# debbiemarkslab/EVcouplings

Hardware: NVIDIA H100
Metric: PLM gradient evals/s as N*L^2*q cell-ops/s (higher is better)
Workload: dtype f32 parameters/accumulation; tensor-core products as bf16 hi+lo pairs (16 mantissa bits)

## Files before the change

evcouplings_b200/csrc/api.cu:

```cuda
#include "../../include/evcplm.h"

#include <stdlib.h>

#include <new>
#include <string>
#include <vector>

#include "common.cuh"
#include "internal.h"

namespace evc {
static thread_local std::string g_err;
void set_error(const std::string &msg) { g_err = msg; }
}

using namespace evc;

static cudaStream_t as_stream(void *s) { return reinterpret_cast<cudaStream_t>(s); }

extern "C" {

int evc_abi_version(void) { return EVCPLM_ABI_VERSION; }

const char *evc_last_error(void) { return g_err.c_str(); }
// ... 241 lines not shown
    float *gJ = d_g + (int64_t)g.L * g.q;
    if ((!tc || (!tcf && !tcff)) && ensure_gather(h)) return 1;
    if (prof) EVC_CUDA(cudaEventRecord(h->ev[0], st));
    if (tcff) {
        if (plm_tcff_expand(g, h->tcff, d_x, h->d_wp_hi, h->d_wp_lo, single, st)) return 1;
        if (prof) EVC_CUDA(cudaEventRecord(h->ev[1], st));
        if (plm_tcff_forward(g, h->tcff, h->tcff_maps, d_x, h->d_msa4, h->d_wts, h->d_rt_hi, h->d_rt_lo, h->tc.Kp,
                             h->d_gh_part3, h->d_fx_part3, single, st))
            return 1;
        if (prof) {
            EVC_CUDA(cudaEventRecord(h->ev[2], st));
            EVC_CUDA(cudaEventRecord(h->ev[3], st));
        }
        if (plm_tc_backward(g, h->tc, h->tc_maps, h->d_Gd, single, st)) return 1;
        if (prof) EVC_CUDA(cudaEventRecord(h->ev[4], st));
        if (plm_tc_finalize_pairs(g, h->tc, h->d_Gd, gJ, 1.0f, st)) return 1;
        if (plm_finalize_fields_n(g, h->d_gh_part3, h->d_fx_part3, d_g, d_fx, h->tcff.ntile_part, st)) return 1;
    } else if (tcf) {
        if (plm_tcf_expand(g, h->tcf, d_x, h->d_wt_hi, h->d_wt_lo, single, st)) return 1;
        if (prof) EVC_CUDA(cudaEventRecord(h->ev[1], st));
        if (plm_tcf_logits(g, h->tcf, h->tcf_maps, h->d_zt, single, st)) return 1;
        if (prof) EVC_CUDA(cudaEventRecord(h->ev[2], st));
        if (plm_tcf_softmax(g, h->tcf, h->d_zt, d_x, h->d_msa4, h->d_wts, h->d_rt_hi, rt_lo, h->tc.Kp,
                            h->d_gh_part2, h->d_fx_part2, st))
            return 1;
        if (prof) EVC_CUDA(cudaEventRecord(h->ev[3], st));
        if (plm_tc_backward(g, h->tc, h->tc_maps, h->d_Gd, single, st)) return 1;
        if (prof) EVC_CUDA(cudaEventRecord(h->ev[4], st));
        if (plm_tc_finalize_pairs(g, h->tc, h->d_Gd, gJ, 1.0f, st)) return 1;
        if (plm_finalize_fields_n(g, h->d_gh_part2, h->d_fx_part2, d_g, d_fx, h->tcf.ntiles_s, st)) return 1;
    } else {
        if (plm_expand(g, d_x, h->d_W, st)) return 1;
        if (!tc) EVC_CUDA(cudaMemsetAsync(h->d_G, 0, (size_t)g.w_floats() * sizeof(float), st));
        if (prof) EVC_CUDA(cudaEventRecord(h->ev[1], st));
        if (plm_forward(g, h->d_W, d_x, h->d_msa4, h->d_wts, h->d_R, tc ? h->d_rt_hi : nullptr,
                        tc ? h->d_rt_lo : nullptr, h->tc.Kp, h->d_gh_part, h->d_fx_part, st))
            return 1;
        if (prof) {
            EVC_CUDA(cudaEventRecord(h->ev[2], st));
            EVC_CUDA(cudaEventRecord(h->ev[3], st));
        }
        if (tc) {
            if (plm_tc_backward(g, h->tc, h->tc_maps, h->d_Gd, single, st)) return 1;
            if (prof) EVC_CUDA(cudaEventRecord(h->ev[4], st));
            if (plm_tc_finalize_pairs(g, h->tc, h->d_Gd, gJ, 1.0f, st)) return 1;
            if (plm_finalize_fields(g, h->d_gh_part, h->d_fx_part, d_g, d_fx, st)) return 1;
        } else {
            if (plm_backward(g, h->d_R, h->d_perm, h->d_bstart, h->d_G, st)) return 1;
            if (prof) EVC_CUDA(cudaEventRecord(h->ev[4], st));
            if (plm_finalize(g, h->d_G, h->d_gh_part, h->d_fx_part, d_g, gJ, d_fx, 1.0f, st)) return 1;
        }
    }
    if (prof) {
        EVC_CUDA(cudaEventRecord(h->ev[5], st));
        h->ev_valid = true;
    }
    return 0;
}

int evc_plm_set_backward(evc_plm_t *h, int32_t mode)
{
    if (!h) { set_error("evc_plm_set_backward: null handle"); return 1; }
    if (mode != 0 && mode != 1) { set_error("evc_plm_set_backward: mode must be 0 (gather) or 1 (tensor core)"); return 1; }
    EVC_CUDA(cudaSetDevice(h->device));
    if (mode == 1 && !h->d_xt) {
        plm_tc_geometry(h->g, h->tc);
        const PlmTcGeom &t = h->tc;
        const size_t xb = (size_t)t.Mp * t.Kp * 2, rb = (size_t)t.Np * t.Kp * 2;
        if (cudaMalloc(&h->d_xt, xb) != cudaSuccess || cudaMalloc(&h->d_rt_hi, rb) != cudaSuccess ||
            cudaMalloc(&h->d_rt_lo, rb) != cudaSuccess ||
            cudaMalloc(&h->d_Gd, (size_t)t.Mp * t.Np * sizeof(float)) != cudaSuccess) {
            set_error(std::string("evc_plm_set_backward: device allocation failed: ") +
                      cudaGetErrorString(cudaGetLastError()));
            return 1;
        }
        EVC_CUDA(cudaMemset(h->d_rt_hi, 0, rb));
        EVC_CUDA(cudaMemset(h->d_rt_lo, 0, rb));
        EVC_CUDA(cudaMemset(h->d_Gd, 0, (size_t)t.Mp * t.Np * sizeof(float)));
        if (plm_tc_build_xt(h->g, t, h->d_msa4, h->d_xt, 0)) return 1;
        EVC_CUDA(cudaDeviceSynchronize());
        h->tc_maps = aligned_alloc(64, round_up((int64_t)plm_tc_map_bytes(), 64));
        if (!h->tc_maps) { set_error("evc_plm_set_backward: out of host memory"); return 1; }
        if (plm_tc_make_maps(t, h->d_xt, h->d_rt_hi, h->d_rt_lo, h->tc_maps)) return 1;
    }
    h->bwd_mode = mode;
    return 0;
}

int evc_plm_set_forward(evc_plm_t *h, int32_t mode)
{
    if (!h) { set_error("evc_plm_set_forward: null handle"); return 1; }
    if (mode < 0 || mode > 2) {
        set_error("evc_plm_set_forward: mode must be 0 (gather), 1 (tensor core) or 2 (tensor core, fused softmax)");
// ... 100 lines not shown
    EVC_CUDA(cudaStreamSynchronize(0));
    return 0;
}

int evc_plm_weighted_counts(evc_plm_t *h, float *d_fi_counts, float *d_fij_counts, void *stream)
{
    if (!h || !d_fi_counts || !d_fij_counts) { set_error("evc_plm_weighted_counts: null pointer"); return 1; }
    cudaStream_t st = as_stream(stream);
    const PlmGeom &g = h->g;
    if (h->bwd_mode == 1 && h->d_gh_part2) {
        const int ntiles = h->tcf.ntiles_s;
        if (plm_tc_onehot_residual(g, ntiles, h->d_msa4, h->d_wts, h->d_rt_hi, h->d_rt_lo, h->tc.Kp, h->d_gh_part2,
                                   h->d_fx_part2, st))
            return 1;
        if (plm_tc_backward(g, h->tc, h->tc_maps, h->d_Gd, 0, st)) return 1;
        if (plm_tc_finalize_pairs(g, h->tc, h->d_Gd, d_fij_counts, 0.5f, st)) return 1;
        return plm_finalize_fields_n(g, h->d_gh_part2, nullptr, d_fi_counts, nullptr, ntiles, st);
    }
    if (ensure_gather(h)) return 1;
    EVC_CUDA(cudaMemsetAsync(h->d_G, 0, (size_t)g.w_floats() * sizeof(float), st));
    if (plm_onehot_residual(g, h->d_msa4, h->d_wts, h->d_R, h->d_gh_part, st)) return 1;
    if (plm_backward(g, h->d_R, h->d_perm, h->d_bstart, h->d_G, st)) return 1;
    return plm_finalize(g, h->d_G, h->d_gh_part, nullptr, d_fi_counts, d_fij_counts, nullptr, 0.5f, st);
}

int evc_ec_scores(const float *d_J_tri, const float *d_fij_tri, const float *d_fi, int32_t L, int32_t q,
                  float *d_fn_raw, float *d_fn_zero_sum, float *d_mi, void *stream)
{
    if (!d_J_tri) { set_error("evc_ec_scores: null pointer"); return 1; }
    return ec_scores(d_J_tri, d_fij_tri, d_fi, L, q, d_fn_raw, d_fn_zero_sum, d_mi, as_stream(stream));
}
// ... 47 lines not shown
```

evcouplings_b200/csrc/internal.h:

```cpp
#pragma once
#include <cuda_runtime.h>
#include <stdint.h>

namespace evc {

int64_t hamming_plane_words(int64_t N, int L);
int64_t hamming_num_tiles(int64_t N);
int hamming_pack(const uint8_t *d_codes, int64_t N, int L, uint32_t *d_planes, cudaStream_t st);
int hamming_count_tiles(const uint32_t *d_planes, int64_t N, int L, int min_identical,
                        int64_t tile_begin, int64_t tile_end, int *d_counts, cudaStream_t st);

int identities_to_seq(const uint8_t *d_codes, const uint8_t *d_seq, int64_t N, int L, int *d_out, cudaStream_t st);

struct PlmGeom {
    int64_t N;
    int L;
    int Lp;
    int q;
    int QB;
    int S;
    int gap_code;
    int64_t Nr;
    int64_t Nld;
    int L4;
// ... 19 lines not shown
                const float *d_wts, float *d_R, void *d_rt_hi, void *d_rt_lo, int64_t Kp, float *d_gh_part,
                double *d_fx_part, cudaStream_t st);
int plm_onehot_residual(const PlmGeom &g, const uint32_t *d_msa4, const float *d_wts, float *d_R,
                        float *d_gh_part, cudaStream_t st);
int plm_backward(const PlmGeom &g, const float *d_R, const uint32_t *d_perm, const uint16_t *d_bstart,
                 float *d_G, cudaStream_t st);
int plm_finalize(const PlmGeom &g, const float *d_G, const float *d_gh_part, const double *d_fx_part,
                 float *d_gh, float *d_gJ, double *d_fx, float scale_pair, cudaStream_t st);
int plm_add_reg(const PlmGeom &g, const float *d_x, float *d_g, double *d_fx, float lambda_h,
                float lambda_J, cudaStream_t st);

struct PlmTcGeom {
    int64_t Mp;
    int64_t Np;
    int64_t Kp;
};
void plm_tc_geometry(const PlmGeom &g, PlmTcGeom &t);
size_t plm_tc_map_bytes();
int plm_tc_build_xt(const PlmGeom &g, const PlmTcGeom &t, const uint32_t *d_msa4, void *d_xt, cudaStream_t st);
int plm_tc_make_maps(const PlmTcGeom &t, void *d_xt, void *d_rt_hi, void *d_rt_lo, void *maps_out_host);
int plm_tc_backward(const PlmGeom &g, const PlmTcGeom &t, const void *maps_host, float *d_Gd, int single,
                    cudaStream_t st);
int plm_tc_onehot_residual(const PlmGeom &g, int ntiles, const uint32_t *d_msa4, const float *d_wts, void *d_rt_hi,
                           void *d_rt_lo, int64_t Kp, float *d_gh_part, double *d_fx_part, cudaStream_t st);
int plm_tc_finalize_pairs(const PlmGeom &g, const PlmTcGeom &t, const float *d_Gd, float *d_gJ, float scale,
                          cudaStream_t st);
struct PlmTcfGeom {
    int64_t Mp;
    int64_t Kw;
    int64_t Ns;
    int64_t Xrows;
    int ntiles_s;
};
void plm_tcf_geometry(const PlmGeom &g, PlmTcfGeom &t);
int plm_tcf_build_x(const PlmGeom &g, const PlmTcfGeom &t, const uint32_t *d_msa4, void *d_x1h, cudaStream_t st);
int plm_tcf_make_maps(const PlmTcfGeom &t, void *d_wt_hi, void *d_wt_lo, void *d_x1h, void *maps_out_host);
int plm_tcf_expand(const PlmGeom &g, const PlmTcfGeom &t, const float *d_x, void *d_wt_hi, void *d_wt_lo,
                   int single, cudaStream_t st);
int plm_tcf_logits(const PlmGeom &g, const PlmTcfGeom &t, const void *maps_host, float *d_zt, int single,
                   cudaStream_t st);
int plm_tcf_softmax(const PlmGeom &g, const PlmTcfGeom &t, const float *d_zt, const float *d_x,
// ... 88 lines not shown
```

evcouplings_b200/csrc/plm_tc.cu:

```cuda
#include <cuda.h>
#include <cuda_bf16.h>

#include <stdlib.h>

#include <algorithm>

#include "common.cuh"
#include "internal.h"

namespace evc {

constexpr int TC_BM = 128;
constexpr int TC_BN = 192;
constexpr int TC_BK = 64;
constexpr int TC_MAX_STAGES = 8;
constexpr int TC_A_BYTES = TC_BM * TC_BK * 2;
constexpr int TC_B_BYTES = TC_BN * TC_BK * 2;
constexpr int TC_SMEM_LIMIT = 232448;
constexpr int TC_SMEM_HEAD = 2048;
constexpr int TC_THREADS = 384;
constexpr int TC_CONSUMERS = 256;
constexpr int TC_K_CHUNK = 32;
constexpr int TC_REG_PRODUCER = 40;
constexpr int TC_REG_CONSUMER = 232;

__device__ __forceinline__ void mbar_wait_bounded(uint64_t *bar, uint32_t parity)
{
    uint32_t done = 0;
    for (uint64_t it = 0; it < (1ull << 31); it++) {
        asm volatile(
            "{\n.reg .pred p;\n"
            "mbarrier.try_wait.parity.shared::cta.b64 p, [%1], %2;\n"
            "selp.u32 %0, 1, 0, p;\n}\n"
            : "=r"(done)
            : "r"(smem_u32(bar)), "r"(parity)
            : "memory");
        if (done) return;
// ... 188 lines not shown
{
    if (threadIdx.x == 0) {
        for (int s = 0; s < n_stages; s++) {
            mbar_init(&l.full[s], 1);
            mbar_init(&l.empty[s], TC_CONSUMERS);
        }
        mbar_fence_init();
    }
    __syncthreads();
}

template <int SPLIT_A, int SINGLE>
__global__ void __launch_bounds__(TC_THREADS, 1)
tc_gemm_kernel(const __grid_constant__ CUtensorMap tm0, const __grid_constant__ CUtensorMap tm1,
               const __grid_constant__ CUtensorMap tm2, float *__restrict__ D, int64_t ldd, int m_tiles, int n_tiles,
               int num_kb, int k_chunk, int mgroup, int n_stages)
{
    constexpr int BYTES0 = TC_A_BYTES;
    constexpr int BYTES1 = TC_B_BYTES;
    constexpr int BYTES2 = SPLIT_A ? TC_A_BYTES : TC_B_BYTES;
    constexpr int stage_bytes = BYTES0 + BYTES1 + (SINGLE ? 0 : BYTES2);
    extern __shared__ unsigned char smem_dyn[];
    const TcSmem l = tc_smem_layout(smem_dyn);
    int m_tile, n_tile;
    decode_tile(blockIdx.x, m_tiles, n_tiles, mgroup, m_tile, n_tile);
    tc_init_barriers(l, n_stages);

    if (threadIdx.x < 128) {
        setmaxnreg_dec<TC_REG_PRODUCER>();
        if (threadIdx.x == 0) {
            const uint64_t keep = l2_policy_evict_last();
            int s = 0;
            uint32_t ph = 0;
            for (int kb = 0; kb < num_kb; kb++) {
                mbar_wait_bounded(&l.empty[s], ph ^ 1u);
                unsigned char *st = l.ring + s * stage_bytes;
                mbar_expect_tx(&l.full[s], (uint32_t)stage_bytes);
                if (SPLIT_A) {
                    tma_load_2d_hint(st, &tm0, kb * TC_BK, m_tile * TC_BM, &l.full[s], keep);
                    tma_load_2d(st + BYTES0, &tm2, kb * TC_BK, n_tile * TC_BN, &l.full[s]);
                    if (!SINGLE) tma_load_2d_hint(st + BYTES0 + BYTES1, &tm1, kb * TC_BK, m_tile * TC_BM, &l.full[s], keep);
                } else {
                    tma_load_2d(st, &tm0, kb * TC_BK, m_tile * TC_BM, &l.full[s]);
                    tma_load_2d(st + BYTES0, &tm1, kb * TC_BK, n_tile * TC_BN, &l.full[s]);
                    if (!SINGLE) tma_load_2d(st + BYTES0 + BYTES1, &tm2, kb * TC_BK, n_tile * TC_BN, &l.full[s]);
                }
                if (++s == n_stages) { s = 0; ph ^= 1u; }
            }
        }
    } else {
        setmaxnreg_inc<TC_REG_CONSUMER>();
        const int cw = (threadIdx.x >> 7) - 1;
        constexpr uint64_t OFF1 = (uint64_t)(BYTES0 >> 4), OFF2 = (uint64_t)((BYTES0 + BYTES1) >> 4);
        const uint64_t arow = (uint64_t)((cw * 64 * TC_BK * 2) >> 4);
        const uint64_t desc0 = make_desc_sw128(l.ring);
        float acc[TC_BN / 2], sum[TC_BN / 2];
#pragma unroll
        for (int u = 0; u < TC_BN / 2; u++) acc[u] = 0.f;
        const int n_chunks = (num_kb + k_chunk - 1) / k_chunk;
        int s = 0;
        uint32_t ph = 0;
        for (int c = 0; c < n_chunks; c++) {
            const int kb0 = c * k_chunk, kb1 = min(num_kb, kb0 + k_chunk);
            if (SPLIT_A) tc_mainloop<TC_BN>(acc, l.full, l.empty, s, ph, n_stages, stage_bytes, kb0, kb1, desc0,
                                            arow, OFF1, OFF2 + arow, OFF1, !SINGLE);
            else tc_mainloop<TC_BN>(acc, l.full, l.empty, s, ph, n_stages, stage_bytes, kb0, kb1, desc0,
                                    arow, OFF1, arow, OFF2, !SINGLE);
#pragma unroll
            for (int u = 0; u < TC_BN / 2; u++) sum[u] = (c == 0) ? acc[u] : sum[u] + acc[u];
        }
        const int t = threadIdx.x & 127;
        const int64_t row = (int64_t)m_tile * TC_BM + cw * 64 + (t >> 5) * 16 + ((t & 31) >> 2);
        float *out = D + row * ldd + (int64_t)n_tile * TC_BN + 2 * (t & 3);
#pragma unroll
        for (int c8 = 0; c8 < TC_BN / 8; c8++) {
            __stcs(reinterpret_cast<float2 *>(out + 8 * c8), make_float2(sum[4 * c8], sum[4 * c8 + 1]));
            __stcs(reinterpret_cast<float2 *>(out + 8 * ldd + 8 * c8), make_float2(sum[4 * c8 + 2], sum[4 * c8 + 3]));
        }
    }
}

constexpr int TF_BN = 176;
constexpr int TF_SITES = 8;
constexpr int TF_B_BYTES = TF_BN * TC_BK * 2;
constexpr int TF_PITCH = TF_BN + 1;

template <int SINGLE>
__global__ void __launch_bounds__(TC_THREADS, 1)
// ... 97 lines not shown
                if (n < g.N) {
                    const int64_t off = ((int64_t)i * q + a) * Kp + n;
                    const __nv_bfloat16 hi = __float2bfloat16_rn(rr);
                    Rt_hi[off] = hi;
                    if (!SINGLE) Rt_lo[off] = __float2bfloat16_rn(rr - __bfloat162float(hi));
                }
            }
            const float tot = warp_sum(rr);
            if (lane == 0) ghp[a] = (a < q) ? tot : 0.f;
        }
        const double fw = warp_sum(fx_local);
        if (lane == 0) fx_part[(int64_t)i * ntile_part + m_tile * 4 + quad] = fw;
    }
}

__global__ void expand_tcf_kernel(const float *__restrict__ x, __nv_bfloat16 *__restrict__ Wp_hi,
                                  __nv_bfloat16 *__restrict__ Wp_lo, int L, int q, int64_t ldw, int single)
{
    const int i = blockIdx.y, j = blockIdx.x;
    if (j <= i) return;
    const float *J = x + (int64_t)L * q + ((int64_t)i * (2 * L - i - 1) / 2 + (j - i - 1)) * q * q;
    const int64_t ri = (int64_t)(i / TF_SITES) * TF_BN + ((i % TF_SITES) / 4) * 88 + (i % 4) * 21;
    const int64_t rj = (int64_t)(j / TF_SITES) * TF_BN + ((j % TF_SITES) / 4) * 88 + (j % 4) * 21;
    for (int e = threadIdx.x; e < q * q; e += blockDim.x) {
        const int a = e / q, b = e - a * q;
        const float v = J[e];
        const __nv_bfloat16 hi = __float2bfloat16_rn(v);
        const __nv_bfloat16 lo = __float2bfloat16_rn(v - __bfloat162float(hi));
        const int64_t p1 = (ri + a) * ldw + (j * q + b);
        const int64_t p2 = (rj + b) * ldw + (i * q + a);
        Wp_hi[p1] = hi;
        Wp_hi[p2] = hi;
        if (!single) { Wp_lo[p1] = lo; Wp_lo[p2] = lo; }
    }
}

__global__ void expand_tc_kernel(const float *__restrict__ x, __nv_bfloat16 *__restrict__ Wt_hi,
                                 __nv_bfloat16 *__restrict__ Wt_lo, int L, int q, int64_t ldw, int single)
{
    const int i = blockIdx.y, j = blockIdx.x;
    if (j <= i) return;
    const float *J = x + (int64_t)L * q + ((int64_t)i * (2 * L - i - 1) / 2 + (j - i - 1)) * q * q;
    for (int e = threadIdx.x; e < q * q; e += blockDim.x) {
        const int a = e / q, b = e - a * q;
        const float v = J[e];
        const __nv_bfloat16 hi = __float2bfloat16_rn(v);
        const __nv_bfloat16 lo = __float2bfloat16_rn(v - __bfloat162float(hi));
        const int64_t p1 = (int64_t)(i * q + a) * ldw + (j * q + b);
        const int64_t p2 = (int64_t)(j * q + b) * ldw + (i * q + a);
        Wt_hi[p1] = hi;
        Wt_hi[p2] = hi;
        if (!single) { Wt_lo[p1] = lo; Wt_lo[p2] = lo; }
    }
}

__global__ void build_x_kernel(const uint32_t *__restrict__ msa4, __nv_bfloat16 *__restrict__ X, int64_t N,
                               int64_t Nld, int L, int q, int64_t ldx)
{
    const int64_t n = blockIdx.x;
    if (n >= N) return;
    for (int e = threadIdx.x; e < L * q; e += blockDim.x) {
        const int j = e / q, b = e - j * q;
        const int code = (int)((msa4[(int64_t)(j >> 2) * Nld + n] >> (8 * (j & 3))) & 0xffu);
        X[n * ldx + e] = __float2bfloat16(code == b ? 1.0f : 0.0f);
    }
}

template <int Q, bool ONEHOT>
// ... 74 lines not shown
    if (tid == 0) fx_part[(int64_t)i * ntiles + tile] = (s_fx[0] + s_fx[1]) + (s_fx[2] + s_fx[3]);
}

__global__ void build_xt_kernel(const uint32_t *__restrict__ msa4, __nv_bfloat16 *__restrict__ Xt, int64_t N,
                                int64_t Nld, int64_t Kp, int L, int q)
{
    const int64_t n = (int64_t)blockIdx.x * blockDim.x + threadIdx.x;
    const int j = blockIdx.y;
    if (n >= Kp) return;
    int code = 255;
    if (n < N) code = (int)((msa4[(int64_t)(j >> 2) * Nld + n] >> (8 * (j & 3))) & 0xffu);
    for (int b = 0; b < q; b++)
        Xt[((int64_t)j * q + b) * Kp + n] = __float2bfloat16(code == b ? 1.0f : 0.0f);
}

__global__ void finalize_pairs_tc_kernel(const float *__restrict__ Gd, float *__restrict__ gJ, int L, int q,
                                         int Np, float scale)
{
    const int i = blockIdx.y, j = blockIdx.x;
    if (j <= i) return;
    float *out = gJ + ((int64_t)i * (2 * L - i - 1) / 2 + (j - i - 1)) * q * q;
    for (int e = threadIdx.x; e < q * q; e += blockDim.x) {
        const int a = e / q, b = e - a * q;
        const float v1 = Gd[(int64_t)(j * q + b) * Np + (i * q + a)];
        const float v2 = Gd[(int64_t)(i * q + a) * Np + (j * q + b)];
        out[e] = scale * (v1 + v2);
    }
}

static int env_int_once(const char *name, int *cache)
{
    if (*cache == -2) {
        const char *e = getenv(name);
        *cache = e ? atoi(e) : -1;
    }
    return *cache;
}

static int stages_for(int stage_bytes)
{
    return std::max(2, std::min(TC_MAX_STAGES, (TC_SMEM_LIMIT - TC_SMEM_HEAD) / stage_bytes));
// ... 19 lines not shown
static int make_map(CUtensorMap *m, void *base, int64_t rows, int64_t kp, int box_rows)
{
    PFN_encodeTiled fn = get_encode_fn();
    if (!fn) { set_error("cuTensorMapEncodeTiled entry point not available"); return 1; }
    cuuint64_t gdim[2] = {(cuuint64_t)kp, (cuuint64_t)rows};
    cuuint64_t gstride[1] = {(cuuint64_t)kp * 2};
    cuuint32_t box[2] = {(cuuint32_t)TC_BK, (cuuint32_t)box_rows};
    cuuint32_t estr[2] = {1, 1};
    CUresult r = fn(m, CU_TENSOR_MAP_DATA_TYPE_BFLOAT16, 2, base, gdim, gstride, box, estr,
                    CU_TENSOR_MAP_INTERLEAVE_NONE, CU_TENSOR_MAP_SWIZZLE_128B, CU_TENSOR_MAP_L2_PROMOTION_L2_256B,
                    CU_TENSOR_MAP_FLOAT_OOB_FILL_NONE);
    if (r != CUDA_SUCCESS) { set_error("cuTensorMapEncodeTiled failed with code " + std::to_string((int)r)); return 1; }
    return 0;
}

void plm_tc_geometry(const PlmGeom &g, PlmTcGeom &t)
{
    const int64_t lq = (int64_t)g.L * g.q;
    t.Mp = round_up(lq, TC_BM);
    t.Np = round_up(lq, TC_BN);
    t.Kp = round_up(g.N, TC_BK);
}

int plm_tc_build_xt(const PlmGeom &g, const PlmTcGeom &t, const uint32_t *d_msa4, void *d_xt, cudaStream_t st)
{
    EVC_CUDA(cudaMemsetAsync(d_xt, 0, (size_t)t.Mp * t.Kp * 2, st));
    dim3 grid((unsigned)ceil_div(t.Kp, 256), (unsigned)g.L);
    build_xt_kernel<<<grid, 256, 0, st>>>(d_msa4, reinterpret_cast<__nv_bfloat16 *>(d_xt), g.N, g.Nld, t.Kp, g.L,
                                          g.q);
    EVC_KERNEL_CHECK();
    return 0;
}

int plm_tc_make_maps(const PlmTcGeom &t, void *d_xt, void *d_rt_hi, void *d_rt_lo, void *maps_out)
{
    CUtensorMap *m = reinterpret_cast<CUtensorMap *>(maps_out);
    if (make_map(&m[0], d_xt, t.Mp, t.Kp, TC_BM)) return 1;
    if (make_map(&m[1], d_rt_hi, t.Np, t.Kp, TC_BN)) return 1;
    if (make_map(&m[2], d_rt_lo, t.Np, t.Kp, TC_BN)) return 1;
    return 0;
}

int plm_tc_backward(const PlmGeom &g, const PlmTcGeom &t, const void *maps, float *d_Gd, int single, cudaStream_t st)
{
    const CUtensorMap *m = reinterpret_cast<const CUtensorMap *>(maps);
    const int stage = TC_A_BYTES + TC_B_BYTES + (single ? 0 : TC_B_BYTES);
    const int n_stages = stages_for(stage);
    const size_t smem = (size_t)n_stages * stage + TC_SMEM_HEAD;
    static int kc_env = -2;
    const int kc = env_int_once("EVC_KCHUNK", &kc_env);
    const int m_tiles = (int)(t.Mp / TC_BM), n_tiles = (int)(t.Np / TC_BN);
    const int grid = m_tiles * n_tiles;
    if (single) {
        EVC_CUDA(cudaFuncSetAttribute(tc_gemm_kernel<0, 1>, cudaFuncAttributeMaxDynamicSharedMemorySize, TC_SMEM_LIMIT));
        tc_gemm_kernel<0, 1><<<grid, TC_THREADS, smem, st>>>(m[0], m[1], m[2], d_Gd, t.Np, m_tiles, n_tiles,
                                                            (int)(t.Kp / TC_BK), kc > 0 ? kc : TC_K_CHUNK, m_tiles,
                                                            n_stages);
    } else {
        EVC_CUDA(cudaFuncSetAttribute(tc_gemm_kernel<0, 0>, cudaFuncAttributeMaxDynamicSharedMemorySize, TC_SMEM_LIMIT));
        tc_gemm_kernel<0, 0><<<grid, TC_THREADS, smem, st>>>(m[0], m[1], m[2], d_Gd, t.Np, m_tiles, n_tiles,
                                                            (int)(t.Kp / TC_BK), kc > 0 ? kc : TC_K_CHUNK, m_tiles,
                                                            n_stages);
    }
    EVC_KERNEL_CHECK();
    return 0;
}

int plm_tc_finalize_pairs(const PlmGeom &g, const PlmTcGeom &t, const float *d_Gd, float *d_gJ, float scale,
                          cudaStream_t st)
{
    dim3 grid((unsigned)g.L, (unsigned)g.L);
    finalize_pairs_tc_kernel<<<grid, 128, 0, st>>>(d_Gd, d_gJ, g.L, g.q, (int)t.Np, scale);
    EVC_KERNEL_CHECK();
    return 0;
}

void plm_tcf_geometry(const PlmGeom &g, PlmTcfGeom &t)
{
    const int64_t lq = (int64_t)g.L * g.q;
    t.Mp = round_up(lq, TC_BM);
    t.Kw = round_up(lq, TC_BK);
    t.Ns = round_up(g.N, TC_BN);
    t.Xrows = round_up(g.N, 384);
    t.ntiles_s = (int)ceil_div(g.N, 256);
}

int plm_tcf_build_x(const PlmGeom &g, const PlmTcfGeom &t, const uint32_t *d_msa4, void *d_x1h, cudaStream_t st)
// ... 5 lines not shown
    return 0;
}

int plm_tcf_make_maps(const PlmTcfGeom &t, void *d_wt_hi, void *d_wt_lo, void *d_x1h, void *maps_out)
{
    CUtensorMap *m = reinterpret_cast<CUtensorMap *>(maps_out);
    if (make_map(&m[0], d_wt_hi, t.Mp, t.Kw, TC_BM)) return 1;
    if (make_map(&m[1], d_wt_lo, t.Mp, t.Kw, TC_BM)) return 1;
    if (make_map(&m[2], d_x1h, t.Xrows, t.Kw, TC_BN)) return 1;
    return 0;
}

int plm_tcf_expand(const PlmGeom &g, const PlmTcfGeom &t, const float *d_x, void *d_wt_hi, void *d_wt_lo,
                   int single, cudaStream_t st)
{
    dim3 grid((unsigned)g.L, (unsigned)g.L);
    expand_tc_kernel<<<grid, 128, 0, st>>>(d_x, reinterpret_cast<__nv_bfloat16 *>(d_wt_hi),
                                          reinterpret_cast<__nv_bfloat16 *>(d_wt_lo), g.L, g.q, t.Kw, single);
    EVC_KERNEL_CHECK();
    return 0;
}

static int forward_mgroup(const PlmTcfGeom &t, int single, int m_tiles)
{
    static int mg_env = -2;
    const int e = env_int_once("EVC_MGROUP", &mg_env);
    if (e > 0) return std::min(e, m_tiles);
    static int mb_env = -2;
    const int mb = env_int_once("EVC_MGROUP_MB", &mb_env);
    const double budget = (mb > 0 ? mb : 24) * 1.0e6;
    const double per_tile = (double)TC_BM * (double)t.Kw * 2.0 * (single ? 1.0 : 2.0);
    return std::max(1, std::min(m_tiles, (int)(budget / per_tile)));
}

int plm_tcf_logits(const PlmGeom &g, const PlmTcfGeom &t, const void *maps, float *d_zt, int single, cudaStream_t st)
{
    const CUtensorMap *m = reinterpret_cast<const CUtensorMap *>(maps);
    const int stage = TC_A_BYTES + TC_B_BYTES + (single ? 0 : TC_A_BYTES);
    const int n_stages = stages_for(stage);
    const size_t smem = (size_t)n_stages * stage + TC_SMEM_HEAD;
    const int m_tiles = (int)(t.Mp / TC_BM), n_tiles = (int)(t.Ns / TC_BN);
    const int num_kb = (int)(t.Kw / TC_BK);
    const int grid = m_tiles * n_tiles;
    const int kchunk = num_kb <= 128 ? num_kb : TC_K_CHUNK;
    const int mgroup = forward_mgroup(t, single, m_tiles);
    if (single) {
        EVC_CUDA(cudaFuncSetAttribute(tc_gemm_kernel<1, 1>, cudaFuncAttributeMaxDynamicSharedMemorySize, TC_SMEM_LIMIT));
        tc_gemm_kernel<1, 1><<<grid, TC_THREADS, smem, st>>>(m[0], m[1], m[2], d_zt, t.Ns, m_tiles, n_tiles, num_kb,
                                                            kchunk, mgroup, n_stages);
    } else {
        EVC_CUDA(cudaFuncSetAttribute(tc_gemm_kernel<1, 0>, cudaFuncAttributeMaxDynamicSharedMemorySize, TC_SMEM_LIMIT));
        tc_gemm_kernel<1, 0><<<grid, TC_THREADS, smem, st>>>(m[0], m[1], m[2], d_zt, t.Ns, m_tiles, n_tiles, num_kb,
                                                            kchunk, mgroup, n_stages);
    }
    EVC_KERNEL_CHECK();
    return 0;
}

template <bool ONEHOT>
static int launch_softmax(const PlmGeom &g, int ntiles, const float *d_zt, int64_t ldz, const float *d_x,
                          const uint32_t *d_msa4, const float *d_wts, __nv_bfloat16 *hi, __nv_bfloat16 *lo,
                          int64_t Kp, float *d_gh_part, double *d_fx_part, cudaStream_t st)
{
    dim3 grid((unsigned)ntiles, (unsigned)g.L);
    switch (g.q) {
        case 21: plm_softmax_kernel<21, ONEHOT><<<grid, 128, 0, st>>>(d_zt, ldz, d_x, d_msa4, d_wts, hi, lo, Kp, d_gh_part, d_fx_part, g, ntiles); break;
        case 20: plm_softmax_kernel<20, ONEHOT><<<grid, 128, 0, st>>>(d_zt, ldz, d_x, d_msa4, d_wts, hi, lo, Kp, d_gh_part, d_fx_part, g, ntiles); break;
        case 5: plm_softmax_kernel<5, ONEHOT><<<grid, 128, 0, st>>>(d_zt, ldz, d_x, d_msa4, d_wts, hi, lo, Kp, d_gh_part, d_fx_part, g, ntiles); break;
// ... 33 lines not shown

bool plm_tcff_supported(const PlmGeom &g) { return g.S == 21; }

int plm_tcff_make_maps(const PlmTcffGeom &t, void *d_x1h, void *d_wp_hi, void *d_wp_lo, void *maps_out)
{
    CUtensorMap *m = reinterpret_cast<CUtensorMap *>(maps_out);
    if (make_map(&m[0], d_x1h, t.Xrows, t.Kw, TC_BM)) return 1;
    if (make_map(&m[1], d_wp_hi, t.Np, t.Kw, TF_BN)) return 1;
    if (make_map(&m[2], d_wp_lo, t.Np, t.Kw, TF_BN)) return 1;
    return 0;
}

int plm_tcff_expand(const PlmGeom &g, const PlmTcffGeom &t, const float *d_x, void *d_wp_hi, void *d_wp_lo,
                    int single, cudaStream_t st)
{
    dim3 grid((unsigned)g.L, (unsigned)g.L);
    expand_tcf_kernel<<<grid, 128, 0, st>>>(d_x, reinterpret_cast<__nv_bfloat16 *>(d_wp_hi),
                                           reinterpret_cast<__nv_bfloat16 *>(d_wp_lo), g.L, g.q, t.Kw, single);
    EVC_KERNEL_CHECK();
    return 0;
}

int plm_tcff_forward(const PlmGeom &g, const PlmTcffGeom &t, const void *maps, const float *d_x,
                     const uint32_t *d_msa4, const float *d_wts, void *d_rt_hi, void *d_rt_lo, int64_t Kp,
                     float *d_gh_part, double *d_fx_part, int single, cudaStream_t st)
{
    const CUtensorMap *m = reinterpret_cast<const CUtensorMap *>(maps);
    const int stage = TC_A_BYTES + TF_B_BYTES + (single ? 0 : TF_B_BYTES);
    const int n_stages = stages_for(stage);
    const size_t smem = (size_t)n_stages * stage + TC_SMEM_HEAD;
    const int grid = t.m_tiles * t.n_tiles;
    auto kernel = single ? tc_fwd_fused_kernel<1> : tc_fwd_fused_kernel<0>;
    EVC_CUDA(cudaFuncSetAttribute(kernel, cudaFuncAttributeMaxDynamicSharedMemorySize, TC_SMEM_LIMIT));
// ... 11 lines not shown
```

Measured before the change: 4395 billion.

## Add split-K backward GEMM and tile-based expand/finalize kernels

Measured after the change: 4570 billion (median of 6 runs). 4.0% higher.

```diff
diff --git a/evcouplings_b200/csrc/api.cu b/evcouplings_b200/csrc/api.cu
--- a/evcouplings_b200/csrc/api.cu
+++ b/evcouplings_b200/csrc/api.cu
@@ -279,7 +279,7 @@
         }
         if (plm_tc_backward(g, h->tc, h->tc_maps, h->d_Gd, single, st)) return 1;
         if (prof) EVC_CUDA(cudaEventRecord(h->ev[4], st));
-        if (plm_tc_finalize_pairs(g, h->tc, h->d_Gd, gJ, 1.0f, st)) return 1;
+        if (plm_tc_finalize_pairs(g, h->tc, h->d_Gd, h->tc.ksplit, gJ, 1.0f, st)) return 1;
         if (plm_finalize_fields_n(g, h->d_gh_part3, h->d_fx_part3, d_g, d_fx, h->tcff.ntile_part, st)) return 1;
     } else if (tcf) {
         if (plm_tcf_expand(g, h->tcf, d_x, h->d_wt_hi, h->d_wt_lo, single, st)) return 1;
@@ -292,7 +292,7 @@
         if (prof) EVC_CUDA(cudaEventRecord(h->ev[3], st));
         if (plm_tc_backward(g, h->tc, h->tc_maps, h->d_Gd, single, st)) return 1;
         if (prof) EVC_CUDA(cudaEventRecord(h->ev[4], st));
-        if (plm_tc_finalize_pairs(g, h->tc, h->d_Gd, gJ, 1.0f, st)) return 1;
+        if (plm_tc_finalize_pairs(g, h->tc, h->d_Gd, h->tc.ksplit, gJ, 1.0f, st)) return 1;
         if (plm_finalize_fields_n(g, h->d_gh_part2, h->d_fx_part2, d_g, d_fx, h->tcf.ntiles_s, st)) return 1;
     } else {
         if (plm_expand(g, d_x, h->d_W, st)) return 1;
@@ -308,7 +308,7 @@
         if (tc) {
             if (plm_tc_backward(g, h->tc, h->tc_maps, h->d_Gd, single, st)) return 1;
             if (prof) EVC_CUDA(cudaEventRecord(h->ev[4], st));
-            if (plm_tc_finalize_pairs(g, h->tc, h->d_Gd, gJ, 1.0f, st)) return 1;
+            if (plm_tc_finalize_pairs(g, h->tc, h->d_Gd, h->tc.ksplit, gJ, 1.0f, st)) return 1;
             if (plm_finalize_fields(g, h->d_gh_part, h->d_fx_part, d_g, d_fx, st)) return 1;
         } else {
             if (plm_backward(g, h->d_R, h->d_perm, h->d_bstart, h->d_G, st)) return 1;
@@ -329,19 +329,21 @@
     if (mode != 0 && mode != 1) { set_error("evc_plm_set_backward: mode must be 0 (gather) or 1 (tensor core)"); return 1; }
     EVC_CUDA(cudaSetDevice(h->device));
     if (mode == 1 && !h->d_xt) {
-        plm_tc_geometry(h->g, h->tc);
+        int sm_count = 0;
+        EVC_CUDA(cudaDeviceGetAttribute(&sm_count, cudaDevAttrMultiProcessorCount, h->device));
+        plm_tc_geometry(h->g, sm_count, h->tc);
         const PlmTcGeom &t = h->tc;
         const size_t xb = (size_t)t.Mp * t.Kp * 2, rb = (size_t)t.Np * t.Kp * 2;
+        const size_t gdb = (size_t)t.ksplit * t.Mp * t.Np * sizeof(float);
         if (cudaMalloc(&h->d_xt, xb) != cudaSuccess || cudaMalloc(&h->d_rt_hi, rb) != cudaSuccess ||
-            cudaMalloc(&h->d_rt_lo, rb) != cudaSuccess ||
-            cudaMalloc(&h->d_Gd, (size_t)t.Mp * t.Np * sizeof(float)) != cudaSuccess) {
+            cudaMalloc(&h->d_rt_lo, rb) != cudaSuccess || cudaMalloc(&h->d_Gd, gdb) != cudaSuccess) {
             set_error(std::string("evc_plm_set_backward: device allocation failed: ") +
                       cudaGetErrorString(cudaGetLastError()));
             return 1;
         }
         EVC_CUDA(cudaMemset(h->d_rt_hi, 0, rb));
         EVC_CUDA(cudaMemset(h->d_rt_lo, 0, rb));
-        EVC_CUDA(cudaMemset(h->d_Gd, 0, (size_t)t.Mp * t.Np * sizeof(float)));
+        EVC_CUDA(cudaMemset(h->d_Gd, 0, gdb));
         if (plm_tc_build_xt(h->g, t, h->d_msa4, h->d_xt, 0)) return 1;
         EVC_CUDA(cudaDeviceSynchronize());
         h->tc_maps = aligned_alloc(64, round_up((int64_t)plm_tc_map_bytes(), 64));
@@ -472,7 +474,7 @@
                                    h->d_fx_part2, st))
             return 1;
         if (plm_tc_backward(g, h->tc, h->tc_maps, h->d_Gd, 0, st)) return 1;
-        if (plm_tc_finalize_pairs(g, h->tc, h->d_Gd, d_fij_counts, 0.5f, st)) return 1;
+        if (plm_tc_finalize_pairs(g, h->tc, h->d_Gd, h->tc.ksplit, d_fij_counts, 0.5f, st)) return 1;
         return plm_finalize_fields_n(g, h->d_gh_part2, nullptr, d_fi_counts, nullptr, ntiles, st);
     }
     if (ensure_gather(h)) return 1;
diff --git a/evcouplings_b200/csrc/internal.h b/evcouplings_b200/csrc/internal.h
--- a/evcouplings_b200/csrc/internal.h
+++ b/evcouplings_b200/csrc/internal.h
@@ -57,8 +57,9 @@
     int64_t Mp;
     int64_t Np;
     int64_t Kp;
+    int ksplit;
 };
-void plm_tc_geometry(const PlmGeom &g, PlmTcGeom &t);
+void plm_tc_geometry(const PlmGeom &g, int sm_count, PlmTcGeom &t);
 size_t plm_tc_map_bytes();
 int plm_tc_build_xt(const PlmGeom &g, const PlmTcGeom &t, const uint32_t *d_msa4, void *d_xt, cudaStream_t st);
 int plm_tc_make_maps(const PlmTcGeom &t, void *d_xt, void *d_rt_hi, void *d_rt_lo, void *maps_out_host);
@@ -66,8 +67,8 @@
                     cudaStream_t st);
 int plm_tc_onehot_residual(const PlmGeom &g, int ntiles, const uint32_t *d_msa4, const float *d_wts, void *d_rt_hi,
                            void *d_rt_lo, int64_t Kp, float *d_gh_part, double *d_fx_part, cudaStream_t st);
-int plm_tc_finalize_pairs(const PlmGeom &g, const PlmTcGeom &t, const float *d_Gd, float *d_gJ, float scale,
-                          cudaStream_t st);
+int plm_tc_finalize_pairs(const PlmGeom &g, const PlmTcGeom &t, const float *d_Gd, int planes, float *d_gJ,
+                          float scale, cudaStream_t st);
 struct PlmTcfGeom {
     int64_t Mp;
     int64_t Kw;
diff --git a/evcouplings_b200/csrc/plm_tc.cu b/evcouplings_b200/csrc/plm_tc.cu
--- a/evcouplings_b200/csrc/plm_tc.cu
+++ b/evcouplings_b200/csrc/plm_tc.cu
@@ -21,6 +21,7 @@
 constexpr int TC_THREADS = 384;
 constexpr int TC_CONSUMERS = 256;
 constexpr int TC_K_CHUNK = 32;
+constexpr int TC_MAX_KSPLIT = 8;
 constexpr int TC_REG_PRODUCER = 40;
 constexpr int TC_REG_CONSUMER = 232;
 
@@ -239,7 +240,7 @@
 __global__ void __launch_bounds__(TC_THREADS, 1)
 tc_gemm_kernel(const __grid_constant__ CUtensorMap tm0, const __grid_constant__ CUtensorMap tm1,
                const __grid_constant__ CUtensorMap tm2, float *__restrict__ D, int64_t ldd, int m_tiles, int n_tiles,
-               int num_kb, int k_chunk, int mgroup, int n_stages)
+               int num_kb, int k_chunk, int mgroup, int n_stages, int ksplit, int64_t plane)
 {
     constexpr int BYTES0 = TC_A_BYTES;
     constexpr int BYTES1 = TC_B_BYTES;
@@ -247,8 +248,12 @@
     constexpr int stage_bytes = BYTES0 + BYTES1 + (SINGLE ? 0 : BYTES2);
     extern __shared__ unsigned char smem_dyn[];
     const TcSmem l = tc_smem_layout(smem_dyn);
+    const int tiles = m_tiles * n_tiles;
+    const int slice = (int)blockIdx.x / tiles;
     int m_tile, n_tile;
-    decode_tile(blockIdx.x, m_tiles, n_tiles, mgroup, m_tile, n_tile);
+    decode_tile((int)blockIdx.x - slice * tiles, m_tiles, n_tiles, mgroup, m_tile, n_tile);
+    const int kb_per = (num_kb + ksplit - 1) / ksplit;
+    const int kb_begin = slice * kb_per, kb_end = min(num_kb, kb_begin + kb_per);
     tc_init_barriers(l, n_stages);
 
     if (threadIdx.x < 128) {
@@ -257,7 +262,7 @@
             const uint64_t keep = l2_policy_evict_last();
             int s = 0;
             uint32_t ph = 0;
-            for (int kb = 0; kb < num_kb; kb++) {
+            for (int kb = kb_begin; kb < kb_end; kb++) {
                 mbar_wait_bounded(&l.empty[s], ph ^ 1u);
                 unsigned char *st = l.ring + s * stage_bytes;
                 mbar_expect_tx(&l.full[s], (uint32_t)stage_bytes);
@@ -282,11 +287,11 @@
         float acc[TC_BN / 2], sum[TC_BN / 2];
 #pragma unroll
         for (int u = 0; u < TC_BN / 2; u++) acc[u] = 0.f;
-        const int n_chunks = (num_kb + k_chunk - 1) / k_chunk;
+        const int n_chunks = (kb_end - kb_begin + k_chunk - 1) / k_chunk;
         int s = 0;
         uint32_t ph = 0;
         for (int c = 0; c < n_chunks; c++) {
-            const int kb0 = c * k_chunk, kb1 = min(num_kb, kb0 + k_chunk);
+            const int kb0 = kb_begin + c * k_chunk, kb1 = min(kb_end, kb0 + k_chunk);
             if (SPLIT_A) tc_mainloop<TC_BN>(acc, l.full, l.empty, s, ph, n_stages, stage_bytes, kb0, kb1, desc0,
                                             arow, OFF1, OFF2 + arow, OFF1, !SINGLE);
             else tc_mainloop<TC_BN>(acc, l.full, l.empty, s, ph, n_stages, stage_bytes, kb0, kb1, desc0,
@@ -296,7 +301,7 @@
         }
         const int t = threadIdx.x & 127;
         const int64_t row = (int64_t)m_tile * TC_BM + cw * 64 + (t >> 5) * 16 + ((t & 31) >> 2);
-        float *out = D + row * ldd + (int64_t)n_tile * TC_BN + 2 * (t & 3);
+        float *out = D + slice * plane + row * ldd + (int64_t)n_tile * TC_BN + 2 * (t & 3);
 #pragma unroll
         for (int c8 = 0; c8 < TC_BN / 8; c8++) {
             __stcs(reinterpret_cast<float2 *>(out + 8 * c8), make_float2(sum[4 * c8], sum[4 * c8 + 1]));
@@ -424,44 +429,86 @@
     }
 }
 
-__global__ void expand_tcf_kernel(const float *__restrict__ x, __nv_bfloat16 *__restrict__ Wp_hi,
-                                  __nv_bfloat16 *__restrict__ Wp_lo, int L, int q, int64_t ldw, int single)
-{
-    const int i = blockIdx.y, j = blockIdx.x;
-    if (j <= i) return;
-    const float *J = x + (int64_t)L * q + ((int64_t)i * (2 * L - i - 1) / 2 + (j - i - 1)) * q * q;
-    const int64_t ri = (int64_t)(i / TF_SITES) * TF_BN + ((i % TF_SITES) / 4) * 88 + (i % 4) * 21;
-    const int64_t rj = (int64_t)(j / TF_SITES) * TF_BN + ((j % TF_SITES) / 4) * 88 + (j % 4) * 21;
-    for (int e = threadIdx.x; e < q * q; e += blockDim.x) {
-        const int a = e / q, b = e - a * q;
-        const float v = J[e];
-        const __nv_bfloat16 hi = __float2bfloat16_rn(v);
-        const __nv_bfloat16 lo = __float2bfloat16_rn(v - __bfloat162float(hi));
-        const int64_t p1 = (ri + a) * ldw + (j * q + b);
-        const int64_t p2 = (rj + b) * ldw + (i * q + a);
-        Wp_hi[p1] = hi;
-        Wp_hi[p2] = hi;
-        if (!single) { Wp_lo[p1] = lo; Wp_lo[p2] = lo; }
-    }
-}
-
-__global__ void expand_tc_kernel(const float *__restrict__ x, __nv_bfloat16 *__restrict__ Wt_hi,
-                                 __nv_bfloat16 *__restrict__ Wt_lo, int L, int q, int64_t ldw, int single)
-{
-    const int i = blockIdx.y, j = blockIdx.x;
-    if (j <= i) return;
-    const float *J = x + (int64_t)L * q + ((int64_t)i * (2 * L - i - 1) / 2 + (j - i - 1)) * q * q;
-    for (int e = threadIdx.x; e < q * q; e += blockDim.x) {
-        const int a = e / q, b = e - a * q;
-        const float v = J[e];
-        const __nv_bfloat16 hi = __float2bfloat16_rn(v);
-        const __nv_bfloat16 lo = __float2bfloat16_rn(v - __bfloat162float(hi));
-        const int64_t p1 = (int64_t)(i * q + a) * ldw + (j * q + b);
-        const int64_t p2 = (int64_t)(j * q + b) * ldw + (i * q + a);
-        Wt_hi[p1] = hi;
-        Wt_hi[p2] = hi;
-        if (!single) { Wt_lo[p1] = lo; Wt_lo[p2] = lo; }
-    }
+constexpr int EXP_SITES = 4;
+constexpr int EXP_THREADS = 256;
+
+template <bool PADDED>
+__device__ __forceinline__ int64_t expand_row(int i, int a, int q)
+{
+    if (PADDED) return (int64_t)(i / TF_SITES) * TF_BN + ((i % TF_SITES) / 4) * 88 + (i % 4) * 21 + a;
+    return (int64_t)i * q + a;
+}
+
+__device__ __forceinline__ void cp_async4(void *smem_dst, const void *gmem_src)
+{
+    asm volatile("cp.async.ca.shared.global [%0], [%1], 4;" ::"r"(smem_u32(smem_dst)), "l"(gmem_src) : "memory");
+}
+__device__ __forceinline__ void cp_async_wait_all() { asm volatile("cp.async.wait_all;" ::: "memory"); }
+
+template <bool PADDED>
+__global__ void __launch_bounds__(EXP_THREADS)
+expand_tc_kernel(const float *__restrict__ x, __nv_bfloat16 *__restrict__ W_hi, __nv_bfloat16 *__restrict__ W_lo,
+                 int L, int q, int64_t ldw, int single)
+{
+    __shared__ float sJ[EXP_SITES * EXP_SITES * 21 * 21];
+    const int ti = blockIdx.y, tj = blockIdx.x;
+    if (tj < ti) return;
+    const int i0 = ti * EXP_SITES, j0 = tj * EXP_SITES;
+    const int ni = min(EXP_SITES, L - i0), nj = min(EXP_SITES, L - j0);
+    const int qq = q * q;
+    for (int ii = 0; ii < ni; ii++) {
+        const int i = i0 + ii, jlo = max(j0, i + 1);
+        if (jlo >= j0 + nj) continue;
+        const float *src = x + (int64_t)L * q + ((int64_t)i * (2 * L - i - 1) / 2 + (jlo - i - 1)) * qq;
+        float *dst = sJ + (ii * EXP_SITES + (jlo - j0)) * qq;
+        const int n = (j0 + nj - jlo) * qq;
+        for (int e = threadIdx.x; e < n; e += blockDim.x) cp_async4(dst + e, src + e);
+    }
+    cp_async_wait_all();
+    __syncthreads();
+    const int lane = threadIdx.x & 31, warp = threadIdx.x >> 5;
+    auto write_tile = [&](int r0, int nr, int c0, int nc) {
+        const int width = nc * q;
+        int csite[4], colN[4], colT[4];
+#pragma unroll
+        for (int k = 0; k < 4; k++) {
+            const int c = 2 * lane + 64 * (k >> 1) + (k & 1);
+            const int cs = c / q, cb = c - cs * q;
+            csite[k] = c0 + cs;
+            colN[k] = cs * qq + cb;
+            colT[k] = cs * EXP_SITES * qq + cb * q;
+        }
+        for (int rr = warp; rr < nr * q; rr += EXP_THREADS / 32) {
+            const int rs = rr / q, ra = rr - rs * q, r = r0 + rs;
+            const int rowN = rs * EXP_SITES * qq + ra * q, rowT = rs * qq + ra;
+            const int64_t off = expand_row<PADDED>(r, ra, q) * ldw + (int64_t)c0 * q;
+            auto elem = [&](int k) -> float {
+                if (r < csite[k]) return sJ[rowN + colN[k]];
+                if (r > csite[k]) return sJ[rowT + colT[k]];
+                return 0.f;
+            };
+#pragma unroll
+            for (int h = 0; h < 2; h++) {
+                const int c = 2 * lane + 64 * h;
+                if (c >= width) continue;
+                const float v0 = elem(2 * h);
+                const __nv_bfloat16 h0 = __float2bfloat16_rn(v0);
+                const __nv_bfloat16 l0 = __float2bfloat16_rn(v0 - __bfloat162float(h0));
+                if (c + 1 < width) {
+                    const float v1 = elem(2 * h + 1);
+                    const __nv_bfloat16 h1 = __float2bfloat16_rn(v1);
+                    const __nv_bfloat16 l1 = __float2bfloat16_rn(v1 - __bfloat162float(h1));
+                    *reinterpret_cast<__nv_bfloat162 *>(W_hi + off + c) = __halves2bfloat162(h0, h1);
+                    if (!single) *reinterpret_cast<__nv_bfloat162 *>(W_lo + off + c) = __halves2bfloat162(l0, l1);
+                } else {
+                    W_hi[off + c] = h0;
+                    if (!single) W_lo[off + c] = l0;
+                }
+            }
+        }
+    };
+    write_tile(i0, ni, j0, nj);
+    if (ti != tj) write_tile(j0, nj, i0, ni);
 }
 
 __global__ void build_x_kernel(const uint32_t *__restrict__ msa4, __nv_bfloat16 *__restrict__ X, int64_t N,
@@ -566,17 +613,77 @@
         Xt[((int64_t)j * q + b) * Kp + n] = __float2bfloat16(code == b ? 1.0f : 0.0f);
 }
 
-__global__ void finalize_pairs_tc_kernel(const float *__restrict__ Gd, float *__restrict__ gJ, int L, int q,
-                                         int Np, float scale)
-{
-    const int i = blockIdx.y, j = blockIdx.x;
-    if (j <= i) return;
-    float *out = gJ + ((int64_t)i * (2 * L - i - 1) / 2 + (j - i - 1)) * q * q;
-    for (int e = threadIdx.x; e < q * q; e += blockDim.x) {
-        const int a = e / q, b = e - a * q;
-        const float v1 = Gd[(int64_t)(j * q + b) * Np + (i * q + a)];
-        const float v2 = Gd[(int64_t)(i * q + a) * Np + (j * q + b)];
-        out[e] = scale * (v1 + v2);
+constexpr int FIN_SITES = 4;
+constexpr int FIN_W = FIN_SITES * 21;
+constexpr int FIN_PITCH = FIN_W + 1;
+constexpr int FIN_THREADS = 256;
+constexpr int FIN_SMEM = 2 * FIN_W * FIN_PITCH * (int)sizeof(float);
+constexpr int FIN_BATCH = 8;
+
+__global__ void __launch_bounds__(FIN_THREADS)
+finalize_pairs_tc_kernel(const float *__restrict__ Gd, int planes, int64_t plane, float *__restrict__ gJ, int L,
+                         int q, int Np, float scale)
+{
+    extern __shared__ float fin_smem[];
+    float *sA = fin_smem;
+    float *sB = fin_smem + FIN_W * FIN_PITCH;
+    const int ti = blockIdx.y, tj = blockIdx.x;
+    if (tj < ti) return;
+    const int i0 = ti * FIN_SITES, j0 = tj * FIN_SITES;
+    const int wi = min(FIN_SITES, L - i0) * q, wj = min(FIN_SITES, L - j0) * q;
+    auto stage = [&](float *dst, int row0, int rows, int col0, int cols) {
+        const int V = (cols % 4 == 0) ? 4 : 1;
+        const int nv = cols / V;
+        const int dr = FIN_THREADS / nv, dc = FIN_THREADS - dr * nv;
+        int r = threadIdx.x / nv, c = threadIdx.x - r * nv;
+        while (r < rows) {
+            float4 v[FIN_BATCH];
+            int off[FIN_BATCH];
+#pragma unroll
+            for (int u = 0; u < FIN_BATCH; u++) {
+                off[u] = r < rows ? r * FIN_PITCH + c * V : -1;
+                if (r < rows) {
+                    const float *p = Gd + (int64_t)(row0 + r) * Np + (col0 + c * V);
+                    v[u] = V == 4 ? *reinterpret_cast<const float4 *>(p) : make_float4(p[0], 0.f, 0.f, 0.f);
+#pragma unroll
+                    for (int s = 1; s < TC_MAX_KSPLIT; s++) {
+                        if (s >= planes) break;
+                        const float *ps = p + s * plane;
+                        const float4 w = V == 4 ? *reinterpret_cast<const float4 *>(ps) : make_float4(ps[0], 0.f, 0.f, 0.f);
+                        v[u].x += w.x; v[u].y += w.y; v[u].z += w.z; v[u].w += w.w;
+                    }
+                }
+                c += dc; r += dr;
+                if (c >= nv) { c -= nv; r++; }
+            }
+#pragma unroll
+            for (int u = 0; u < FIN_BATCH; u++) {
+                if (off[u] < 0) break;
+                float *d = dst + off[u];
+                d[0] = v[u].x;
+                if (V == 4) { d[1] = v[u].y; d[2] = v[u].z; d[3] = v[u].w; }
+            }
+        }
+    };
+    stage(sA, i0 * q, wi, j0 * q, wj);
+    stage(sB, j0 * q, wj, i0 * q, wi);
+    __syncthreads();
+    const int qq = q * q;
+    const int sj = FIN_THREADS / qq, sa = (FIN_THREADS % qq) / q, sb = FIN_THREADS % q;
+    for (int ii = 0; ii * q < wi; ii++) {
+        const int i = i0 + ii, jlo = max(j0, i + 1);
+        const int n = (j0 + wj / q - jlo) * qq;
+        if (n <= 0) continue;
+        float *out = gJ + ((int64_t)i * (2 * L - i - 1) / 2 + (jlo - i - 1)) * qq;
+        int jj = jlo - j0 + threadIdx.x / qq, a = (threadIdx.x % qq) / q, b = threadIdx.x % q;
+        for (int e = threadIdx.x; e < n; e += FIN_THREADS) {
+            const float v1 = sB[(jj * q + b) * FIN_PITCH + ii * q + a];
+            const float v2 = sA[(ii * q + a) * FIN_PITCH + jj * q + b];
+            out[e] = scale * (v1 + v2);
+            b += sb; a += sa; jj += sj;
+            if (b >= q) { b -= q; a++; }
+            if (a >= q) { a -= q; jj++; }
+        }
     }
 }
 
@@ -626,12 +733,33 @@
     return 0;
 }
 
-void plm_tc_geometry(const PlmGeom &g, PlmTcGeom &t)
+static int backward_ksplit(int64_t tiles, int num_kb, int sm_count)
+{
+    static int ks_env = -2;
+    const int e = env_int_once("EVC_KSPLIT", &ks_env);
+    int ks = 1;
+    if (e > 0) {
+        ks = std::min(e, TC_MAX_KSPLIT);
+    } else {
+        double best = 0.0;
+        for (int s = 1; s <= 4 && s <= num_kb; s++) {
+            const int64_t units = tiles * s;
+            const double eff = (double)units / ((double)sm_count * (double)ceil_div(units, sm_count));
+            if (eff >= 0.97) { ks = s; break; }
+            if (eff > best) { best = eff; ks = s; }
+        }
+    }
+    ks = std::max(1, std::min(ks, num_kb));
+    return (int)ceil_div(num_kb, ceil_div(num_kb, ks));
+}
+
+void plm_tc_geometry(const PlmGeom &g, int sm_count, PlmTcGeom &t)
 {
     const int64_t lq = (int64_t)g.L * g.q;
     t.Mp = round_up(lq, TC_BM);
     t.Np = round_up(lq, TC_BN);
     t.Kp = round_up(g.N, TC_BK);
+    t.ksplit = backward_ksplit((t.Mp / TC_BM) * (t.Np / TC_BN), (int)(t.Kp / TC_BK), sm_count);
 }
 
 int plm_tc_build_xt(const PlmGeom &g, const PlmTcGeom &t, const uint32_t *d_msa4, void *d_xt, cudaStream_t st)
@@ -662,27 +790,30 @@
     static int kc_env = -2;
     const int kc = env_int_once("EVC_KCHUNK", &kc_env);
     const int m_tiles = (int)(t.Mp / TC_BM), n_tiles = (int)(t.Np / TC_BN);
-    const int grid = m_tiles * n_tiles;
+    const int grid = m_tiles * n_tiles * t.ksplit;
+    const int64_t plane = t.Mp * t.Np;
     if (single) {
         EVC_CUDA(cudaFuncSetAttribute(tc_gemm_kernel<0, 1>, cudaFuncAttributeMaxDynamicSharedMemorySize, TC_SMEM_LIMIT));
         tc_gemm_kernel<0, 1><<<grid, TC_THREADS, smem, st>>>(m[0], m[1], m[2], d_Gd, t.Np, m_tiles, n_tiles,
                                                             (int)(t.Kp / TC_BK), kc > 0 ? kc : TC_K_CHUNK, m_tiles,
-                                                            n_stages);
+                                                            n_stages, t.ksplit, plane);
     } else {
         EVC_CUDA(cudaFuncSetAttribute(tc_gemm_kernel<0, 0>, cudaFuncAttributeMaxDynamicSharedMemorySize, TC_SMEM_LIMIT));
         tc_gemm_kernel<0, 0><<<grid, TC_THREADS, smem, st>>>(m[0], m[1], m[2], d_Gd, t.Np, m_tiles, n_tiles,
                                                             (int)(t.Kp / TC_BK), kc > 0 ? kc : TC_K_CHUNK, m_tiles,
-                                                            n_stages);
+                                                            n_stages, t.ksplit, plane);
     }
     EVC_KERNEL_CHECK();
     return 0;
 }
 
-int plm_tc_finalize_pairs(const PlmGeom &g, const PlmTcGeom &t, const float *d_Gd, float *d_gJ, float scale,
-                          cudaStream_t st)
-{
-    dim3 grid((unsigned)g.L, (unsigned)g.L);
-    finalize_pairs_tc_kernel<<<grid, 128, 0, st>>>(d_Gd, d_gJ, g.L, g.q, (int)t.Np, scale);
+int plm_tc_finalize_pairs(const PlmGeom &g, const PlmTcGeom &t, const float *d_Gd, int planes, float *d_gJ,
+                          float scale, cudaStream_t st)
+{
+    const unsigned nt = (unsigned)ceil_div(g.L, FIN_SITES);
+    EVC_CUDA(cudaFuncSetAttribute(finalize_pairs_tc_kernel, cudaFuncAttributeMaxDynamicSharedMemorySize, FIN_SMEM));
+    finalize_pairs_tc_kernel<<<dim3(nt, nt), FIN_THREADS, FIN_SMEM, st>>>(d_Gd, planes, t.Mp * t.Np, d_gJ, g.L, g.q,
+                                                                         (int)t.Np, scale);
     EVC_KERNEL_CHECK();
     return 0;
 }
@@ -718,9 +849,10 @@
 int plm_tcf_expand(const PlmGeom &g, const PlmTcfGeom &t, const float *d_x, void *d_wt_hi, void *d_wt_lo,
                    int single, cudaStream_t st)
 {
-    dim3 grid((unsigned)g.L, (unsigned)g.L);
-    expand_tc_kernel<<<grid, 128, 0, st>>>(d_x, reinterpret_cast<__nv_bfloat16 *>(d_wt_hi),
-                                          reinterpret_cast<__nv_bfloat16 *>(d_wt_lo), g.L, g.q, t.Kw, single);
+    const unsigned nt = (unsigned)ceil_div(g.L, EXP_SITES);
+    expand_tc_kernel<false><<<dim3(nt, nt), EXP_THREADS, 0, st>>>(d_x, reinterpret_cast<__nv_bfloat16 *>(d_wt_hi),
+                                                                  reinterpret_cast<__nv_bfloat16 *>(d_wt_lo), g.L, g.q,
+                                                                  t.Kw, single);
     EVC_KERNEL_CHECK();
     return 0;
 }
@@ -751,11 +883,11 @@
     if (single) {
         EVC_CUDA(cudaFuncSetAttribute(tc_gemm_kernel<1, 1>, cudaFuncAttributeMaxDynamicSharedMemorySize, TC_SMEM_LIMIT));
         tc_gemm_kernel<1, 1><<<grid, TC_THREADS, smem, st>>>(m[0], m[1], m[2], d_zt, t.Ns, m_tiles, n_tiles, num_kb,
-                                                            kchunk, mgroup, n_stages);
+                                                            kchunk, mgroup, n_stages, 1, 0);
     } else {
         EVC_CUDA(cudaFuncSetAttribute(tc_gemm_kernel<1, 0>, cudaFuncAttributeMaxDynamicSharedMemorySize, TC_SMEM_LIMIT));
         tc_gemm_kernel<1, 0><<<grid, TC_THREADS, smem, st>>>(m[0], m[1], m[2], d_zt, t.Ns, m_tiles, n_tiles, num_kb,
-                                                            kchunk, mgroup, n_stages);
+                                                            kchunk, mgroup, n_stages, 1, 0);
     }
     EVC_KERNEL_CHECK();
     return 0;
@@ -819,9 +951,10 @@
 int plm_tcff_expand(const PlmGeom &g, const PlmTcffGeom &t, const float *d_x, void *d_wp_hi, void *d_wp_lo,
                     int single, cudaStream_t st)
 {
-    dim3 grid((unsigned)g.L, (unsigned)g.L);
-    expand_tcf_kernel<<<grid, 128, 0, st>>>(d_x, reinterpret_cast<__nv_bfloat16 *>(d_wp_hi),
-                                           reinterpret_cast<__nv_bfloat16 *>(d_wp_lo), g.L, g.q, t.Kw, single);
+    const unsigned nt = (unsigned)ceil_div(g.L, EXP_SITES);
+    expand_tc_kernel<true><<<dim3(nt, nt), EXP_THREADS, 0, st>>>(d_x, reinterpret_cast<__nv_bfloat16 *>(d_wp_hi),
+                                                                 reinterpret_cast<__nv_bfloat16 *>(d_wp_lo), g.L, g.q,
+                                                                 t.Kw, single);
     EVC_KERNEL_CHECK();
     return 0;
 }
```
